# twosigma/Cook

Hardware: AMD Instinct MI355X
Metric: match-cycles/sec at 1M pending x 50k offers (higher is better)
Workload: dtype f64

## Files before the change

cook_amd/csrc/considerable_host.hpp:

```cpp
#pragma once

struct ConsWork {
  DArr<uint64_t> ukey;
  DArr<uint32_t> permA, permB, g_user, seg_start, seg_end, inexact, rate_limited, passed, qitemA, qitemB;
  DArr<uint8_t> head;
  DArr<SumU4> g_use, pre, quseA, quseB, pusage;
  DArr<int> flag1, keep_q;
  DArr<SumI> scan;
  uint32_t* result = nullptr;
  unsigned n_result = 0;
};

struct ConsBufs : ConsWork {
  bool users_staged = false;
  unsigned U = 0;
  DArr<double> qcount, qcpus, qmem, qgpus, ucount, ucpus, umem, ugpus;
  DArr<int64_t> tokens;
  bool has_tokens = false;
  int enforce = 0;
  bool has_pool_quota = false, pool_usage_given = false;
  cook_usage pool_quota{}, pool_usage{};
  bool cycle_on = false;
  DArr<uint8_t> elig_by_pending;
  bool has_elig_by_pending = false;
  DArr<double> q_cpus, q_mem, q_gpus;
  DArr<uint32_t> q_user;
  DArr<uint8_t> q_elig;
};

void cons_stage_users(cook_engine* e, ConsBufs& c, const cook_user_state* us) {
  if (!us) e->fail(COOK_E_INVALID, "cook_considerable: null user state");
  const unsigned U = us->n;
  limiter_check_user_state(e, us);
  if (U && (!us->quota_count || !us->quota_cpus || !us->quota_mem || !us->quota_gpus || !us->usage_count || !us->usage_cpus ||
            !us->usage_mem || !us->usage_gpus))
    e->fail(COOK_E_INVALID, "cook_considerable: user quota / usage arrays are required");
  c.U = U;
  h2d(e, c.qcount, us->quota_count, U);
  h2d(e, c.qcpus, us->quota_cpus, U);
  h2d(e, c.qmem, us->quota_mem, U);
  h2d(e, c.qgpus, us->quota_gpus, U);
  h2d(e, c.ucount, us->usage_count, U);
  h2d(e, c.ucpus, us->usage_cpus, U);
  h2d(e, c.umem, us->usage_mem, U);
  h2d(e, c.ugpus, us->usage_gpus, U);
  c.has_tokens = us->tokens_left != nullptr;
  if (c.has_tokens) h2d(e, c.tokens, us->tokens_left, U);
  c.enforce = us->enforce_rate_limit;
  c.has_pool_quota = us->has_pool_quota != 0;
  c.pool_quota = us->pool_quota;
  c.pool_usage_given = us->pool_usage_given != 0;
  c.pool_usage = us->pool_usage;
  sync(e);
  c.users_staged = true;
}

enum LimUse { LIM_NONE, LIM_CYCLE, LIM_READ };
void cons_run_device(cook_engine* e, const ConsBufs& s, ConsWork& c, unsigned n, const double* q_cpus, const double* q_mem,
                     const double* q_gpus, const uint32_t* q_user, const uint8_t* q_elig, unsigned K, LimUse limiters = LIM_NONE) {
  const unsigned U = s.U;
  const LimView lim = limiters != LIM_NONE ? limiter_view(e, U, limiters == LIM_CYCLE) : LimView{};
  const bool lim_commit = limiters == LIM_CYCLE && lim.tokens;
  c.rate_limited.ensure(std::max(1u, U));
  c.passed.ensure(std::max(1u, U));
  memset_async(e, c.rate_limited.ptr(), 0, (size_t)std::max(1u, U) * 4);
  memset_async(e, c.passed.ptr(), 0, (size_t)std::max(1u, U) * 4);
  c.n_result = 0;
  c.result = c.qitemA.ensure(std::max(1u, n));
  if (n == 0) return;
  const unsigned gN = div_up(n, 256);
  c.ukey.ensure(n);
  c.permA.ensure(n);
  c.permB.ensure(n);
  KM<cons_user_keys, 256>(e, "cons_user_keys", gN, q_user, n, c.ukey.ptr());
  KM<iota_u32, 256>(e, "iota", gN, c.permA.ptr(), n);
  unsigned long long umask = 0;
  for (unsigned long long x = U ? U - 1 : 0; x; x >>= 1) umask = (umask << 1) | 1ull;
  const uint32_t* permU = radix_sort_masked(e, c.ukey.ptr(), umask, c.permA.ptr(), c.permA.ptr(), c.permB.ptr(), n);
  c.g_user.ensure(n);
  c.g_use.ensure(n);
  c.head.ensure(n);
  c.seg_start.ensure(std::max(1u, U));
  c.seg_end.ensure(std::max(1u, U));
  c.inexact.ensure(std::max(1u, U));
  c.pre.ensure(n);
  memset_async(e, c.inexact.ptr(), 0, (size_t)std::max(1u, U) * 4);
  KM<cons_gather, 256>(e, "cons_gather", gN, permU, n, q_user, q_cpus, q_mem, q_gpus, c.g_user.ptr(), c.g_use.ptr(), c.head.ptr(), c.seg_start.ptr(),
      c.seg_end.ptr());
  LoadUserSeeded ld{c.g_use.ptr(), c.head.ptr(), c.g_user.ptr(), s.ucount.ptr(), s.ucpus.ptr(), s.umem.ptr(), s.ugpus.ptr()};
  seg_scan<SumU4>(e, "cons_user_usage_scan", ld, (const uint8_t*)c.head.ptr(), n, c.pre.ptr(), e->tmpU4);
  KM<rank_mark_inexact, 256>(e, "rank_mark_inexact", gN, (const SumU4*)c.pre.ptr(), (const uint32_t*)c.g_user.ptr(), n, c.inexact.ptr());
  KM<cons_fix_inexact, 256>(e, "cons_fix_inexact", div_up(std::max(1u, U), 256), (const SumU4*)c.g_use.ptr(), c.pre.ptr(),
      (const uint32_t*)c.seg_start.ptr(), (const uint32_t*)c.seg_end.ptr(), (const uint32_t*)c.inexact.ptr(), U, (const double*)s.ucount.ptr(),
      (const double*)s.ucpus.ptr(), (const double*)s.umem.ptr(), (const double*)s.ugpus.ptr());
  c.flag1.ensure(n);
  c.keep_q.ensure(n);
  c.scan.ensure(n);
  KM<cons_user_quota_flag, 256>(e, "cons_user_quota_flag", gN, (const SumU4*)c.pre.ptr(), (const uint32_t*)c.g_user.ptr(), n,
      (const double*)s.qcount.ptr(), (const double*)s.qcpus.ptr(), (const double*)s.qmem.ptr(), (const double*)s.qgpus.ptr(), c.flag1.ptr());
  seg_scan<SumI>(e, "cons_user_index_scan", LoadI{c.flag1.ptr()}, (const uint8_t*)c.head.ptr(), n, c.scan.ptr(), e->tmpI);
  unsigned* dlen = e->d_counters.ptr() + LIM_F_LEN;
  const unsigned f_words = lim_commit ? LIM_F_WORDS : 1u;
  memset_async(e, dlen, 0, f_words * 4);
  KM<cons_rate_limit, 256>(e, "cons_rate_limit", gN, (const int*)c.flag1.ptr(), (const SumI*)c.scan.ptr(), (const uint32_t*)c.g_user.ptr(), permU, n,
      s.has_tokens ? (const int64_t*)s.tokens.ptr() : (const int64_t*)nullptr, lim, s.enforce, c.keep_q.ptr(), c.rate_limited.ptr(), c.passed.ptr());
  if (lim_commit) limiter_commit_earn(e, lim, U, c.passed.ptr(), c.rate_limited.ptr(), e->d_counters.ptr());
  uint32_t* qitem = c.qitemA.ensure(n);
  uint32_t* qitem_o = c.qitemB.ensure(n);
  SumU4* quse = c.quseA.ensure(n);
  SumU4* quse_o = c.quseB.ensure(n);
  seg_scan<SumI>(e, "cons_compact_scan", LoadI{c.keep_q.ptr()}, (const uint8_t*)nullptr, n, c.scan.ptr(), e->tmpI);
  KM<cons_compact_queue, 256>(e, "cons_compact_queue", gN, (const int*)c.keep_q.ptr(), (const SumI*)c.scan.ptr(), n, q_cpus, q_mem, q_gpus, qitem, quse, dlen);
  cook_usage base = s.pool_usage;
  if (s.has_pool_quota && !s.pool_usage_given) {
    c.pusage.ensure(1);
    if (U) {
      KM<cons_pool_usage, 1024>(e, "cons_pool_usage", 1, (const double*)s.ucount.ptr(), (const double*)s.ucpus.ptr(), (const double*)s.umem.ptr(),
          (const double*)s.ugpus.ptr(), U, c.pusage.ptr());
      pinned_copy(e, e->h_scratch + 8, c.pusage.ptr(), sizeof(SumU4), hipMemcpyDeviceToHost);
    }
  }
  pinned_copy(e, e->h_scratch, dlen, f_words * 4, hipMemcpyDeviceToHost);
  sync(e);
  unsigned len = 0;
  std::memcpy(&len, e->h_scratch, 4);
  if (lim_commit) limiter_filter_finish(e, (const unsigned*)e->h_scratch);
  if (s.has_pool_quota && !s.pool_usage_given) {
    SumU4 h = SumU4::zero();
    if (U) std::memcpy(&h, e->h_scratch + 8, sizeof(SumU4));
    base = cook_usage{h.count, h.cpus, h.mem, h.gpus};
  }
  if (len && s.has_pool_quota) len = queue_filter_quota(e, 2, len, s.pool_quota, base, qitem, quse, qitem_o, quse_o);
  if (len && q_elig) {
    e->iflag.ensure(len);
    e->scanI.ensure(len);
    KM<cons_eligible_flag, 256>(e, "cons_eligible_flag", div_up(len, 256), (const uint32_t*)qitem, len, q_elig, e->iflag.ptr());
    seg_scan<SumI>(e, "queue_compact_scan", LoadI{e->iflag.ptr()}, (const uint8_t*)nullptr, len, e->scanI.ptr(), e->tmpI);
    unsigned* len_out = e->d_counters.ptr() + 9;
    KM<queue_compact, 256>(e, "queue_compact", div_up(len, 256), (const uint32_t*)qitem, (const SumU4*)quse, (const int*)e->iflag.ptr(),
        (const SumI*)e->scanI.ptr(), len, qitem_o, quse_o, len_out);
    pinned_copy(e, e->h_scratch, len_out, 4, hipMemcpyDeviceToHost);
    sync(e);
    std::memcpy(&len, e->h_scratch, 4);
    std::swap(qitem, qitem_o);
    std::swap(quse, quse_o);
  }
  c.result = qitem;
  c.n_result = std::min(len, K);
}
```

cook_amd/csrc/considerable_kernels.hpp:

```cpp
#pragma once
#include "common.hpp"
#include "scan.hpp"
#include "limiter_kernels.hpp"

COOK_KERNEL void cons_user_keys(const uint32_t* __restrict__ user, unsigned n, uint64_t* __restrict__ key) {
  const unsigned i = blockIdx.x * blockDim.x + threadIdx.x;
  if (i < n) key[i] = user[i];
}

COOK_KERNEL void cons_gather_queue(const uint32_t* __restrict__ ranked, const uint32_t* __restrict__ pend_ord,
                                                         unsigned n, const double* __restrict__ j_cpus, const double* __restrict__ j_mem,
                                                         const double* __restrict__ j_gpus, const uint32_t* __restrict__ j_user,
                                                         const uint8_t* __restrict__ elig_by_pending, double* __restrict__ q_cpus,
                                                         double* __restrict__ q_mem, double* __restrict__ q_gpus,
                                                         uint32_t* __restrict__ q_user, uint8_t* __restrict__ q_elig) {
  const unsigned q = blockIdx.x * blockDim.x + threadIdx.x;
  if (q >= n) return;
  const unsigned jj = pend_ord[ranked[q]];
  q_cpus[q] = j_cpus[jj];
  q_mem[q] = j_mem[jj];
  q_gpus[q] = j_gpus ? j_gpus[jj] : 0.0;
  q_user[q] = j_user[jj];
  q_elig[q] = elig_by_pending ? elig_by_pending[jj] : 1;
}

COOK_KERNEL void cons_gather(const uint32_t* __restrict__ permU, unsigned n, const uint32_t* __restrict__ user,
                                                   const double* __restrict__ cpus, const double* __restrict__ mem,
                                                   const double* __restrict__ gpus, uint32_t* __restrict__ g_user,
                                                   SumU4* __restrict__ g_use, uint8_t* __restrict__ head,
                                                   uint32_t* __restrict__ seg_start, uint32_t* __restrict__ seg_end) {
  const unsigned i = blockIdx.x * blockDim.x + threadIdx.x;
  if (i >= n) return;
  const unsigned t = permU[i];
  const unsigned u = user[t];
  g_user[i] = u;
  g_use[i] = SumU4{1.0, cpus[t], mem[t], gpus ? gpus[t] : 0.0, 0u};
  const bool h = (i == 0) || (user[permU[i - 1]] != u);
  head[i] = h ? 1 : 0;
  if (h) seg_start[u] = i;
  if (i == n - 1 || user[permU[i + 1]] != u) seg_end[u] = i + 1;
}

struct LoadUserSeeded {
  const SumU4* use;
  const uint8_t* head;
  const uint32_t* g_user;
  const double *uc, *ucpus, *umem, *ugpus;
  __device__ __forceinline__ SumU4 operator()(unsigned i) const {
    const SumU4 x = use[i];
    if (!head[i]) return x;
    const unsigned u = g_user[i];
    return combine(x, SumU4{uc[u], ucpus[u], umem[u], ugpus[u], 0u});
  }
};

COOK_KERNEL void cons_fix_inexact(const SumU4* __restrict__ g_use, SumU4* __restrict__ pre,
                                                        const uint32_t* __restrict__ seg_start, const uint32_t* __restrict__ seg_end,
                                                        const uint32_t* __restrict__ inexact_user, unsigned n_users,
                                                        const double* __restrict__ uc, const double* __restrict__ ucpus,
                                                        const double* __restrict__ umem, const double* __restrict__ ugpus) {
// ... 119 lines not shown
```

cook_amd/csrc/rank_host.hpp:

```cpp

template <class T, class Load>
void seg_scan(cook_engine* e, const char* tag, Load load, const uint8_t* head, unsigned n, T* out, ScanTmp<T>& tmp) {
  if (n == 0) return;
  const unsigned nb = div_up(n, SS_TILE);
  tmp.agg.ensure(nb);
  tmp.carry.ensure(nb);
  tmp.first_head.ensure(nb);
  KM<seg_scan_local<T, Load>, SS_THREADS>(e, tag, nb, load, head, n, out, tmp.agg.ptr(), tmp.first_head.ptr());
  if (nb > 1 && nb <= (unsigned)SS_THREADS) {
    KM<seg_scan_propagate_fused<T>, SS_THREADS>(e, "seg_scan_propagate", nb, out, n, (const SegAgg<T>*)tmp.agg.ptr(), (const unsigned*)tmp.first_head.ptr());
  } else if (nb > 1) {
    KM<seg_scan_blocksums<T>, SS_THREADS>(e, "seg_scan_blocksums", 1, (const SegAgg<T>*)tmp.agg.ptr(), nb, tmp.carry.ptr());
    KM<seg_scan_propagate<T>, SS_THREADS>(e, "seg_scan_propagate", nb, out, n, (const SegAgg<T>*)tmp.carry.ptr(), (const unsigned*)tmp.first_head.ptr());
  }
}

template <int IPL>
static void radix_pass_t(cook_engine* e, const uint64_t* key, const uint32_t* in, uint32_t* out, unsigned n, unsigned shift, bool fused,
                         DArr<uint32_t>& hist) {
  const unsigned nb = div_up(n, rs_tile(IPL));
  hist.ensure((size_t)256 * nb);
  KM<radix_hist<IPL>, RS_THREADS>(e, "radix_hist", nb, key, in, n, shift, nb, fused ? 1u : 0u, hist.ptr());
  if (!fused) KM<excl_scan_u32_single, SCAN1_THREADS>(e, "radix_scan", 1, hist.ptr(), 256u * nb, (uint32_t*)nullptr);
  KM<radix_scatter<IPL>, RS_THREADS>(e, "radix_scatter", nb, key, in, out, n, shift, nb, fused ? 1u : 0u, (const uint32_t*)hist.ptr());
}
void radix_pass(cook_engine* e, const uint64_t* key, const uint32_t* in, uint32_t* out, unsigned n, unsigned shift, DArr<uint32_t>& hist) {
  if (div_up(n, rs_tile(RS_IPL_SMALL)) <= RS_FUSED_BLOCKS) radix_pass_t<RS_IPL_SMALL>(e, key, in, out, n, shift, true, hist);
  else radix_pass_t<RS_IPL_LARGE>(e, key, in, out, n, shift, div_up(n, rs_tile(RS_IPL_LARGE)) <= RS_FUSED_BLOCKS_LARGE, hist);
}
uint32_t* radix_sort_masked(cook_engine* e, const uint64_t* key, unsigned long long mask, const uint32_t* cur, uint32_t* a,
                            uint32_t* b, unsigned n, DArr<uint32_t>* hist = nullptr) {
  const uint32_t* in = cur;
  uint32_t* last = const_cast<uint32_t*>(cur);
  while (mask) {
    const unsigned shift = (unsigned)__builtin_ctzll(mask);
    uint32_t* out = (in == a) ? b : a;
    radix_pass(e, key, in, out, n, shift, hist ? *hist : e->hist);
    in = out;
    last = out;
    mask = shift + 8 >= 64 ? 0ull : mask & ~((1ull << (shift + 8)) - 1ull);
  }
  return last;
}

COOK_KERNEL void iota_u32(uint32_t* p, unsigned n) {
  const unsigned i = blockIdx.x * blockDim.x + threadIdx.x;
  if (i < n) p[i] = i;
}

void rank_stage(cook_engine* e, const cook_tasks* t, const cook_users* u) {
  if (!t || !u) e->fail(COOK_E_INVALID, "cook_rank_stage: null tasks/users");
  const unsigned N = t->n, U = u->n;
  if (N && (!t->cpus || !t->mem || !t->user || !t->priority || !t->start_ms || !t->task_id || !t->job_id || !t->pending))
    e->fail(COOK_E_INVALID, "cook_rank_stage: a required task array is NULL");
  if (U == 0 && N) e->fail(COOK_E_INVALID, "cook_rank_stage: no users");
  unsigned np = 0;
  std::vector<uint32_t> pend_ord(N ? N : 1);
  for (unsigned i = 0; i < N; ++i) {
    if (t->user[i] >= U) e->fail(COOK_E_INVALID, "cook_rank_stage: user id out of range");
    pend_ord[i] = np;
    np += t->pending[i] ? 1u : 0u;
  }
  e->rank_staged = false, e->pool_usage_known = false, e->rank_done = false;
  e->hash_set = 0;
  e->N = N;
  e->U = U;
  e->n_pending = np;
  e->has_gpus = t->gpus != nullptr;
  h2d(e, e->t_cpus, t->cpus, N);
  h2d(e, e->t_mem, t->mem, N);
  if (t->gpus) h2d(e, e->t_gpus, t->gpus, N);
  h2d(e, e->t_user, t->user, N);
  h2d(e, e->t_prio, t->priority, N);
  h2d(e, e->t_start, t->start_ms, N);
  h2d(e, e->t_task, t->task_id, N);
  h2d(e, e->t_job, t->job_id, N);
  h2d(e, e->t_pending, t->pending, N);
  e->has_t_host = e->t_host_complete = t->host != nullptr;
  if (t->host) h2d(e, e->t_host, t->host, N);
  h2d(e, e->pend_ord, pend_ord.data(), N);
  h2d(e, e->u_divc, u->div_cpus, U);
  h2d(e, e->u_divm, u->div_mem, U);
  h2d(e, e->u_divg, u->div_gpus, U);
  h2d(e, e->u_qcount, u->quota_count, U);
  h2d(e, e->u_qcpus, u->quota_cpus, U);
  h2d(e, e->u_qmem, u->quota_mem, U);
  h2d(e, e->u_qgpus, u->quota_gpus, U);
  sync(e);
  e->rank_staged = true;
  e->pool_usage_known = false;
  e->rank_done = false;
}

void rank_pool_usage(cook_engine* e, cook_usage* out) {
  if (!e->rank_staged) e->fail(COOK_E_STATE, "cook_rank_pool_usage before cook_rank_stage");
  static const bool memo = [] { const char* v = std::getenv("COOK_POOL_USAGE_MEMO"); return !(v && v[0] == '0'); }();
  if (e->pool_usage_known && memo) {
    *out = e->pool_usage_val;
    return;
  }
  e->pool_usage.ensure(1);
  if (e->N == 0) {
    *out = cook_usage{0, 0, 0, 0};
    return;
  }
  e->pool_usage.ensure(1 + POOL_USAGE_BLOCKS);
  e->pool_usage_bound.ensure(POOL_USAGE_BLOCKS);
  KM<pool_usage_partial, 256>(e, "pool_usage_partial", POOL_USAGE_BLOCKS, (const double*)e->t_cpus.ptr(), (const double*)e->t_mem.ptr(),
      e->has_gpus ? (const double*)e->t_gpus.ptr() : (const double*)nullptr, (const uint8_t*)e->t_pending.ptr(), e->N, e->pool_usage.ptr() + 1,
      e->pool_usage_bound.ptr(), (unsigned)POOL_USAGE_BLOCKS);
  KM<pool_usage_reduce, COOK_WAVE>(e, "pool_usage_reduce", 1, (const double*)e->t_cpus.ptr(), (const double*)e->t_mem.ptr(),
      e->has_gpus ? (const double*)e->t_gpus.ptr() : (const double*)nullptr, (const uint8_t*)e->t_pending.ptr(), e->N,
      (const SumU4*)(e->pool_usage.ptr() + 1), (const SumBound4*)e->pool_usage_bound.ptr(), (unsigned)POOL_USAGE_BLOCKS, e->pool_usage.ptr());
  SumU4 h;
  pinned_copy(e, e->h_scratch, e->pool_usage.ptr(), sizeof(SumU4), hipMemcpyDeviceToHost);
  sync(e);
  std::memcpy(&h, e->h_scratch, sizeof(SumU4));
  *out = cook_usage{h.count, h.cpus, h.mem, h.gpus};
  e->pool_usage_val = *out;
  e->pool_usage_known = true;
}

void rank_user_usage(cook_engine* e, double* out, bool out_is_device) {
  if (!e->rank_done) e->fail(COOK_E_STATE, "cook_rank_user_usage before cook_rank_run");
  if (!out) e->fail(COOK_E_INVALID, "cook_rank_user_usage: null output");
  const unsigned N = e->N, U = e->U;
  if (U == 0) return;
  double* dst = out_is_device ? out : e->uu_out.ensure((size_t)U * 3);
  if (N) {
    SumU4* rp = e->uu_pre.ensure(N);
    uint32_t* bad = e->uu_bad.ensure(U);
    memset_async(e, bad, 0, (size_t)U * 4);
    seg_scan<SumU4>(e, "user_running_scan", LoadRunningU4{e->s_use.ptr(), e->s_pending.ptr()}, (const uint8_t*)e->head.ptr(), N, rp,
                    e->tmpU4);
    KM<rank_mark_inexact, 256>(e, "user_usage_mark", div_up(N, 256), (const SumU4*)rp, (const uint32_t*)e->s_user.ptr(), N, bad);
    KM<user_usage_extract, 256>(e, "user_usage_extract", div_up(U, 256), (const SumU4*)rp, (const SumU4*)e->s_use.ptr(),
        (const uint8_t*)e->s_pending.ptr(), (const uint32_t*)e->seg_start.ptr(), (const uint32_t*)e->seg_end.ptr(), (const uint32_t*)bad, U, dst);
  } else {
    memset_async(e, dst, 0, (size_t)U * 24);
  }
  if (!out_is_device) copy_async(e, out, dst, (size_t)U * 24, hipMemcpyDeviceToHost);
  sync(e);
}

unsigned queue_filter_quota(cook_engine* e, unsigned stage, unsigned len, const cook_usage& quota, const cook_usage& base, uint32_t*& qitem,
                            SumU4*& quse, uint32_t*& qitem_other, SumU4*& quse_other) {
  if (len == 0) return 0;
  e->qpre.ensure(len);
  e->iflag.ensure(len);
  e->scanI.ensure(len);
  LoadQueueUse ld{quse, SumU4{base.count, base.cpus, base.mem, base.gpus, 0u}};
  seg_scan<SumU4>(e, "queue_usage_scan", ld, (const uint8_t*)nullptr, len, e->qpre.ptr(), e->tmpU4);
  unsigned* any_bad = e->d_counters.ptr() + 32 + 2 * stage;
  if (stage >= 2) memset_async(e, any_bad, 0, 8);
  Usage4 q{quota.count, quota.cpus, quota.mem, quota.gpus};
  KM<queue_quota_flag, 256>(e, "queue_quota_flag", div_up(len, 256), (const SumU4*)e->qpre.ptr(), len, q, e->iflag.ptr(), any_bad);
  KM<queue_quota_fix, 64>(e, "queue_quota_fix", 1, (const SumU4*)quse, len, SumU4{base.count, base.cpus, base.mem, base.gpus, 0u}, q,
      (const unsigned*)any_bad, e->iflag.ptr());
  seg_scan<SumI>(e, "queue_compact_scan", LoadI{e->iflag.ptr()}, (const uint8_t*)nullptr, len, e->scanI.ptr(), e->tmpI);
  unsigned* len_out = any_bad + 1;
  KM<queue_compact, 256>(e, "queue_compact", div_up(len, 256), (const uint32_t*)qitem, (const SumU4*)quse, (const int*)e->iflag.ptr(),
      (const SumI*)e->scanI.ptr(), len, qitem_other, quse_other, len_out);
  unsigned h[2];
  pinned_copy(e, e->h_scratch, len_out, 4, hipMemcpyDeviceToHost);
  sync(e);
  std::memcpy(h, e->h_scratch, 4);
  std::swap(qitem, qitem_other);
  std::swap(quse, quse_other);
  return h[0];
}

void rank_run(cook_engine* e) {
  if (!e->rank_staged) e->fail(COOK_E_STATE, "cook_rank_run before cook_rank_stage");
  const auto t_call = std::chrono::steady_clock::now();
  if (g_sync_trace) tl_sync_ms = 0.0, tl_syncs = 0;
  const unsigned N = e->N, U = e->U;
  e->n_ranked = 0;
  e->rank_done = false;
  e->cycle_cons_ran = false;
  e->q_valid = false;
  e->q_stepped = false;
  e->ranked.ensure(std::max(1u, e->n_pending));
  if (N == 0) {
    e->rank_done = true;
    return;
  }
  const unsigned gN = div_up(N, 256);
  e->d_scratch64.ensure(64);
  e->d_counters.ensure(64);
  const bool radix_only = std::getenv("COOK_RANK_RADIX") != nullptr;
  unsigned long long* mins = e->d_scratch64.ptr();
  unsigned long long* same = e->d_scratch64.ptr() + 4;
  e->seg_start.ensure(U);
  e->seg_end.ensure(U);
  e->inexact_user.ensure(U);
  TieCtl* tie_ctl0 = e->tie_ctl.ensure(1);
  bool tie_ctl_clean = true;
  KM<rank_init, 256>(e, "rank_init", std::max(1u, std::min(div_up(U, 256), 64u)), e->d_scratch64.ptr(), e->d_counters.ptr(), 40u,
      e->inexact_user.ptr(), e->seg_end.ptr(), U, reinterpret_cast<unsigned*>(tie_ctl0), (unsigned)(sizeof(TieCtl) / 4), std::max(1u,
      std::min(div_up(U, 256), 64u)));
  e->w0.ensure(N);
  e->w1.ensure(N);
  e->w2.ensure(N);
  KM<rank_key_mins, 256>(e, "rank_key_mins", std::min(gN, 64u), (const int64_t*)e->t_start.ptr(), (const int64_t*)e->t_task.ptr(),
      (const int64_t*)e->t_job.ptr(), (const uint8_t*)e->t_pending.ptr(), N, mins, std::min(gN, 64u));
  KM<rank_build_keys, 256>(e, "rank_build_keys", gN, (const uint32_t*)e->t_user.ptr(), (const int32_t*)e->t_prio.ptr(),
      (const int64_t*)e->t_start.ptr(), (const int64_t*)e->t_task.ptr(), (const int64_t*)e->t_job.ptr(), (const uint8_t*)e->t_pending.ptr(), N,
// ... 235 lines not shown
```

cook_amd/csrc/rank_kernels.hpp:

```cpp
#pragma once
#include "common.hpp"
#include "scan.hpp"

COOK_KERNEL void rank_init(unsigned long long* __restrict__ scratch64, unsigned* __restrict__ counters, unsigned n_counters,
                                                 uint32_t* __restrict__ inexact_user, uint32_t* __restrict__ seg_end, unsigned n_users,
                                                 unsigned* __restrict__ tie_ctl, unsigned tie_ctl_words, unsigned nblk ) {
  const unsigned i = blockIdx.x * blockDim.x + threadIdx.x;
  if (i < 7) scratch64[i] = ~0ull;
  if (i < n_counters) counters[i] = 0u;
  if (i < tie_ctl_words) tie_ctl[i] = 0u;
  for (unsigned u = i; u < n_users; u += nblk * blockDim.x) {
    inexact_user[u] = 0u;
    seg_end[u] = 0u;
  }
}

COOK_KERNEL void rank_key_mins(const int64_t* __restrict__ start_ms, const int64_t* __restrict__ task_id,
                                                     const int64_t* __restrict__ job_id, const uint8_t* __restrict__ pending,
                                                     unsigned n, unsigned long long* __restrict__ mins , unsigned nblk) {
  unsigned long long m0 = ~0ull, m1 = ~0ull, m2 = ~0ull;
  for (unsigned i = blockIdx.x * blockDim.x + threadIdx.x; i < n; i += nblk * blockDim.x) {
    if (pending[i]) {
      const unsigned long long k = i64_key(job_id[i]);
      m1 = k < m1 ? k : m1;
// ... 356 lines not shown
    cp = x.cpus + cp;
    m = x.mem + m;
    g = x.gpus + g;
    flag[q] = below_quota4(quota.count, quota.cpus, quota.mem, quota.gpus, Usage4{c, cp, m, g}) ? 1 : 0;
  }
}

COOK_KERNEL void queue_offensive_flag(const SumU4* __restrict__ quse, unsigned len, double max_mem, double max_cpus,
                                                            int* __restrict__ flag) {
  const unsigned q = blockIdx.x * blockDim.x + threadIdx.x;
  if (q >= len) return;
  const SumU4 x = quse[q];
  flag[q] = (x.mem > max_mem || x.cpus > max_cpus) ? 0 : 1;
}

COOK_KERNEL void queue_compact(const uint32_t* __restrict__ qitem_in, const SumU4* __restrict__ quse_in,
                                                     const int* __restrict__ flag, const SumI* __restrict__ incl, unsigned len,
                                                     uint32_t* __restrict__ qitem_out, SumU4* __restrict__ quse_out,
                                                     unsigned* __restrict__ len_out) {
  const unsigned q = blockIdx.x * blockDim.x + threadIdx.x;
  if (q >= len) return;
  if (flag[q]) {
    const unsigned o = (unsigned)incl[q].v - 1;
    qitem_out[o] = qitem_in[q];
    quse_out[o] = quse_in[q];
  }
  if (q == len - 1) *len_out = (unsigned)incl[q].v;
}

COOK_KERNEL void queue_emit(const uint32_t* __restrict__ qitem, unsigned len, const uint32_t* __restrict__ permB,
                                                  uint32_t* __restrict__ ranked) {
  const unsigned q = blockIdx.x * blockDim.x + threadIdx.x;
  if (q < len) ranked[q] = permB[qitem[q]];
}
COOK_KERNEL void dru_to_task_space(const double* __restrict__ dru, const uint8_t* __restrict__ keep,
                                                         const uint32_t* __restrict__ permB, unsigned n, double* __restrict__ out) {
  const unsigned i = blockIdx.x * blockDim.x + threadIdx.x;
  if (i < n) out[permB[i]] = keep[i] ? dru[i] : __longlong_as_double(0x7FF8000000000000ll);
}

struct LoadRunningU4 {
  const SumU4* use;
  const uint8_t* pending;
  __device__ __forceinline__ SumU4 operator()(unsigned i) const {
    if (pending[i]) return SumU4::zero();
    SumU4 x = use[i];
    if (__double_as_longlong(x.cpus) == LLONG_MIN || __double_as_longlong(x.mem) == LLONG_MIN || __double_as_longlong(x.gpus) == LLONG_MIN)
      x.bad = 1u;
    return x;
  }
};
COOK_KERNEL void user_usage_extract(const SumU4* __restrict__ run_pre, const SumU4* __restrict__ s_use,
                                                          const uint8_t* __restrict__ s_pending, const uint32_t* __restrict__ seg_start,
                                                          const uint32_t* __restrict__ seg_end, const uint32_t* __restrict__ inexact_user,
                                                          unsigned n_users, double* __restrict__ out ) {
  const unsigned u = blockIdx.x * blockDim.x + threadIdx.x;
  if (u >= n_users) return;
  double c = 0.0, m = 0.0, g = 0.0;
  if (seg_end[u] != 0u) {
    const unsigned a = seg_start[u], b = seg_end[u];
    const SumU4 t = run_pre[b - 1];
    if (!inexact_user[u]) {
      c = t.cpus, m = t.mem, g = t.gpus;
    } else {
      bool first = true;
      for (unsigned i = a; i < b; ++i) {
        if (s_pending[i]) continue;
        const SumU4 x = s_use[i];
        if (first) {
          c = x.cpus, m = x.mem, g = x.gpus;
          first = false;
        } else {
          c += x.cpus, m += x.mem, g += x.gpus;
        }
      }
    }
  }
  out[(size_t)u * 3 + 0] = c;
  out[(size_t)u * 3 + 1] = m;
  out[(size_t)u * 3 + 2] = g;
}
constexpr int POOL_USAGE_BLOCKS = 64;
COOK_KERNEL void pool_usage_partial(const double* __restrict__ cpus, const double* __restrict__ mem,
                                                          const double* __restrict__ gpus, const uint8_t* __restrict__ pending,
                                                          unsigned n, SumU4* __restrict__ part, SumBound4* __restrict__ part_bound, unsigned nblk) {
  __shared__ SumU4 ws[256 / COOK_WAVE];
  __shared__ SumBound4 wb[256 / COOK_WAVE];
  SumU4 acc = SumU4::zero();
  SumBound4 bd = SumBound4::zero();
  for (unsigned i = blockIdx.x * blockDim.x + threadIdx.x; i < n; i += nblk * blockDim.x)
    if (!pending[i]) {
      const double x[4] = {1.0, cpus[i], mem[i], gpus ? gpus[i] : 0.0};
      acc = combine(acc, SumU4{x[0], x[1], x[2], x[3], 0u});
      bound_add(bd, x);
    }
  for (int d = 32; d >= 1; d >>= 1) {
    SumU4 o;
    o.count = __shfl_xor(acc.count, d, COOK_WAVE);
    o.cpus = __shfl_xor(acc.cpus, d, COOK_WAVE);
    o.mem = __shfl_xor(acc.mem, d, COOK_WAVE);
    o.gpus = __shfl_xor(acc.gpus, d, COOK_WAVE);
    o.bad = __shfl_xor(acc.bad, d, COOK_WAVE);
    acc = combine(acc, o);
    bound_merge(bd, bound_shfl_xor(bd, d));
  }
  if (lane_id() == 0) ws[wave_id()] = acc, wb[wave_id()] = bd;
  __syncthreads();
  if (threadIdx.x == 0) {
    SumU4 t = ws[0];
    SumBound4 tb = wb[0];
    for (unsigned k = 1; k < blockDim.x / COOK_WAVE; ++k) t = combine(t, ws[k]), bound_merge(tb, wb[k]);
    part[blockIdx.x] = t;
    part_bound[blockIdx.x] = tb;
  }
}
// ... 26 lines not shown
```

cook_amd/csrc/sort.hpp:

```cpp
#pragma once
#include "common.hpp"

constexpr int RS_THREADS = 256;
constexpr int RS_WAVES = RS_THREADS / COOK_WAVE;
constexpr int RS_IPL_LARGE = 16;
constexpr int RS_IPL_SMALL = 8;
constexpr unsigned RS_FUSED_BLOCKS = COOK_SHAPE(128, 2);
constexpr unsigned RS_FUSED_BLOCKS_LARGE = COOK_SHAPE(512, 3);
constexpr unsigned rs_tile(int ipl) { return (unsigned)(RS_WAVES * COOK_WAVE * ipl); }

static __device__ __forceinline__ unsigned rs_digit(const uint64_t* __restrict__ key, const uint32_t* __restrict__ perm_in,
                                                    unsigned i, unsigned shift) {
  const unsigned src = perm_in ? perm_in[i] : i;
  return (unsigned)(key[src] >> shift) & 0xFFu;
}

template <int IPL>
COOK_KERNEL void radix_hist(const uint64_t* __restrict__ key, const uint32_t* __restrict__ perm_in,
                                                         unsigned n, unsigned shift, unsigned nblocks, unsigned fused,
                                                         uint32_t* __restrict__ hist) {
  __shared__ unsigned h[256];
  h[threadIdx.x] = 0;
  __syncthreads();
  const unsigned base = blockIdx.x * rs_tile(IPL);
  unsigned d[rs_tile(IPL) / RS_THREADS];
#pragma unroll
  for (unsigned k = 0; k < rs_tile(IPL) / RS_THREADS; ++k) {
    const unsigned i = base + k * RS_THREADS + threadIdx.x;
    d[k] = i < n ? rs_digit(key, perm_in, i, shift) : 0xFFFFFFFFu;
  }
#pragma unroll
  for (unsigned k = 0; k < rs_tile(IPL) / RS_THREADS; ++k)
    if (d[k] != 0xFFFFFFFFu) atomicAdd(&h[d[k]], 1u);
  __syncthreads();
  hist[fused ? blockIdx.x * 256u + threadIdx.x : threadIdx.x * nblocks + blockIdx.x] = h[threadIdx.x];
}

constexpr int SCAN1_THREADS = 1024;
constexpr int SCAN1_IPT = 8;
constexpr int SCAN1_NS = 8;
static_assert(SCAN1_IPT == 8, "a thread moves its entries as two 16-byte vectors");
COOK_KERNEL void excl_scan_u32_single(uint32_t* __restrict__ data, unsigned len,
                                                                      uint32_t* __restrict__ total_out) {
  __shared__ unsigned wsum[2][SCAN1_THREADS / COOK_WAVE];
  unsigned carry = 0;
  const unsigned lane = lane_id(), w = wave_id();
  constexpr unsigned STEP = SCAN1_THREADS * SCAN1_IPT;
  for (unsigned super = 0; super < len; super += STEP * SCAN1_NS) {
    unsigned v[SCAN1_NS][SCAN1_IPT];
#pragma unroll
    for (int s = 0; s < SCAN1_NS; ++s) {
      const unsigned i0 = super + (unsigned)s * STEP + threadIdx.x * SCAN1_IPT;
      if (i0 + SCAN1_IPT <= len) {
        const uint4 a = *reinterpret_cast<const uint4*>(data + i0), b = *reinterpret_cast<const uint4*>(data + i0 + 4);
        v[s][0] = a.x, v[s][1] = a.y, v[s][2] = a.z, v[s][3] = a.w;
        v[s][4] = b.x, v[s][5] = b.y, v[s][6] = b.z, v[s][7] = b.w;
      } else {
#pragma unroll
        for (int q = 0; q < SCAN1_IPT; ++q) v[s][q] = i0 + q < len ? data[i0 + q] : 0u;
      }
    }
#pragma unroll
    for (int s = 0; s < SCAN1_NS; ++s) {
      if (super + (unsigned)s * STEP >= len) break;
      const unsigned i0 = super + (unsigned)s * STEP + threadIdx.x * SCAN1_IPT;
      unsigned tot = 0;
#pragma unroll
      for (int q = 0; q < SCAN1_IPT; ++q) tot += v[s][q];
      unsigned inc = tot;
      for (unsigned d = 1; d < COOK_WAVE; d <<= 1) {
        const unsigned t = __shfl_up(inc, d, COOK_WAVE);
        if (lane >= d) inc += t;
      }
      if (lane == COOK_WAVE - 1) wsum[s & 1][w] = inc;
      __syncthreads();
      unsigned wbase = 0, all = 0;
      for (unsigned k = 0; k < SCAN1_THREADS / COOK_WAVE; ++k) {
        const unsigned x = wsum[s & 1][k];
        wbase += k < w ? x : 0u;
        all += x;
      }
      unsigned run = carry + wbase + inc - tot;
      unsigned o[SCAN1_IPT];
#pragma unroll
      for (int q = 0; q < SCAN1_IPT; ++q) {
        o[q] = run;
        run += v[s][q];
      }
      if (i0 + SCAN1_IPT <= len) {
        *reinterpret_cast<uint4*>(data + i0) = uint4{o[0], o[1], o[2], o[3]};
        *reinterpret_cast<uint4*>(data + i0 + 4) = uint4{o[4], o[5], o[6], o[7]};
      } else {
#pragma unroll
        for (int q = 0; q < SCAN1_IPT; ++q)
          if (i0 + q < len) data[i0 + q] = o[q];
      }
      carry += all;
    }
  }
  if (total_out && threadIdx.x == 0) *total_out = carry;
}

template <int IPL>
COOK_KERNEL void radix_scatter(const uint64_t* __restrict__ key, const uint32_t* __restrict__ perm_in,
                                                            uint32_t* __restrict__ perm_out, unsigned n, unsigned shift,
                                                            unsigned nblocks, unsigned fused, const uint32_t* __restrict__ hist) {
  __shared__ unsigned whist[RS_WAVES][256];
  __shared__ unsigned wtot[RS_WAVES];
  __shared__ uint4 s_tot[RS_WAVES][COOK_WAVE], s_bel[RS_WAVES][COOK_WAVE];
  const unsigned lane = lane_id(), w = wave_id();
  for (int k = 0; k < RS_WAVES; ++k) whist[k][threadIdx.x] = 0;
  unsigned below = 0, total = 0;
  if (fused) {
    uint4 tot{0u, 0u, 0u, 0u}, bel{0u, 0u, 0u, 0u};
#pragma unroll 8
    for (unsigned t = w; t < nblocks; t += RS_WAVES) {
      const uint4 v = *reinterpret_cast<const uint4*>(hist + (size_t)t * 256u + 4u * lane);
      tot.x += v.x, tot.y += v.y, tot.z += v.z, tot.w += v.w;
      if (t < blockIdx.x) bel.x += v.x, bel.y += v.y, bel.z += v.z, bel.w += v.w;
    }
    s_tot[w][lane] = tot;
    s_bel[w][lane] = bel;
  }
  __syncthreads();
  if (fused) {
    const unsigned* pt = reinterpret_cast<const unsigned*>(&s_tot[0][0]);
    const unsigned* pb = reinterpret_cast<const unsigned*>(&s_bel[0][0]);
    for (int k = 0; k < RS_WAVES; ++k) {
      total += pt[k * 256 + threadIdx.x];
      below += pb[k * 256 + threadIdx.x];
    }
  }
  const unsigned wbase = blockIdx.x * rs_tile(IPL) + w * (COOK_WAVE * IPL);
  unsigned src[IPL], dg[IPL];
#pragma unroll
  for (int k = 0; k < IPL; ++k) {
    const unsigned i = wbase + k * COOK_WAVE + lane;
    src[k] = i < n ? (perm_in ? perm_in[i] : i) : 0xFFFFFFFFu;
  }
#pragma unroll
  for (int k = 0; k < IPL; ++k) dg[k] = src[k] != 0xFFFFFFFFu ? (unsigned)(key[src[k]] >> shift) & 0xFFu : 0u;
#pragma unroll
  for (int k = 0; k < IPL; ++k)
    if (src[k] != 0xFFFFFFFFu) atomicAdd(&whist[w][dg[k]], 1u);
  if (fused) {
    unsigned inc = total;
    for (unsigned d = 1; d < COOK_WAVE; d <<= 1) {
      const unsigned t = __shfl_up(inc, d, COOK_WAVE);
      if (lane >= d) inc += t;
    }
    if (lane == COOK_WAVE - 1) wtot[w] = inc;
    __syncthreads();
    unsigned before = 0;
    for (unsigned k = 0; k < (unsigned)RS_WAVES; ++k) before += k < w ? wtot[k] : 0u;
    below += before + inc - total;
  } else {
    __syncthreads();
    below = hist[threadIdx.x * nblocks + blockIdx.x];
  }
  {
    unsigned base = below;
    for (int k = 0; k < RS_WAVES; ++k) {
      const unsigned t = whist[k][threadIdx.x];
      whist[k][threadIdx.x] = base;
      base += t;
    }
  }
  __syncthreads();
  const unsigned long long lt = lanemask_lt();
#pragma unroll
  for (int k = 0; k < IPL; ++k) {
    const bool valid = src[k] != 0xFFFFFFFFu;
    const unsigned d = dg[k];
    unsigned long long peers = __ballot(valid);
    for (int b = 0; b < 8; ++b) {
      const unsigned long long m = __ballot(valid && ((d >> b) & 1u));
      peers &= ((d >> b) & 1u) ? m : ~m;
    }
    unsigned slot = 0;
    if (valid) slot = whist[w][d];
    wave_sync();
    if (valid) {
      const unsigned rank = (unsigned)__popcll(peers & lt);
      if (rank == 0) whist[w][d] = slot + (unsigned)__popcll(peers);
      perm_out[slot + rank] = src[k];
    }
    wave_sync();
  }
}

COOK_KERNEL void radix_varying_bits(const uint64_t* __restrict__ key, unsigned n,
                                                          unsigned long long* __restrict__ out_mask, unsigned nblk) {
  const uint64_t k0 = key[0];
  unsigned long long m = 0;
  for (unsigned i = blockIdx.x * blockDim.x + threadIdx.x; i < n; i += nblk * blockDim.x) m |= key[i] ^ k0;
  for (int d = 32; d >= 1; d >>= 1) m |= __shfl_xor(m, d, COOK_WAVE);
  __shared__ unsigned long long s_m[256 / COOK_WAVE];
  if (lane_id() == 0) s_m[wave_id()] = m;
  __syncthreads();
  if (threadIdx.x == 0) {
    unsigned long long b = 0ull;
    for (unsigned w = 0; w < blockDim.x / COOK_WAVE; ++w) b |= s_m[w];
    if (b) atomicOr(out_mask, b);
  }
}
```

Measured before the change: 23.07.

## Fold memsets into key kernel, widen radix digits to 9 bits, lazy-clear flags

```diff
diff --git a/cook_amd/csrc/considerable_host.hpp b/cook_amd/csrc/considerable_host.hpp
--- a/cook_amd/csrc/considerable_host.hpp
+++ b/cook_amd/csrc/considerable_host.hpp
@@ -56,6 +56,7 @@
 }
 
 enum LimUse { LIM_NONE, LIM_CYCLE, LIM_READ };
+constexpr unsigned CONS_CLEAR_FROM = 36, CONS_CLEAR_WORDS = 11;
 void cons_run_device(cook_engine* e, const ConsBufs& s, ConsWork& c, unsigned n, const double* q_cpus, const double* q_mem,
                      const double* q_gpus, const uint32_t* q_user, const uint8_t* q_elig, unsigned K, LimUse limiters = LIM_NONE) {
   const unsigned U = s.U;
@@ -63,16 +64,21 @@
   const bool lim_commit = limiters == LIM_CYCLE && lim.tokens;
   c.rate_limited.ensure(std::max(1u, U));
   c.passed.ensure(std::max(1u, U));
-  memset_async(e, c.rate_limited.ptr(), 0, (size_t)std::max(1u, U) * 4);
-  memset_async(e, c.passed.ptr(), 0, (size_t)std::max(1u, U) * 4);
   c.n_result = 0;
   c.result = c.qitemA.ensure(std::max(1u, n));
-  if (n == 0) return;
+  if (n == 0) {
+    memset_async(e, c.rate_limited.ptr(), 0, (size_t)std::max(1u, U) * 4);
+    memset_async(e, c.passed.ptr(), 0, (size_t)std::max(1u, U) * 4);
+    return;
+  }
   const unsigned gN = div_up(n, 256);
   c.ukey.ensure(n);
   c.permA.ensure(n);
   c.permB.ensure(n);
-  KM<cons_user_keys, 256>(e, "cons_user_keys", gN, q_user, n, c.ukey.ptr());
+  c.inexact.ensure(std::max(1u, U));
+  static_assert(CONS_CLEAR_FROM + CONS_CLEAR_WORDS == LIM_F_LEN + LIM_F_WORDS && CONS_CLEAR_WORDS <= 256, "one thread per cleared counter");
+  KM<cons_user_keys, 256>(e, "cons_user_keys", gN, q_user, n, c.ukey.ptr(), c.rate_limited.ptr(), c.passed.ptr(), c.inexact.ptr(), std::max(1u, U),
+      e->d_counters.ptr() + CONS_CLEAR_FROM, CONS_CLEAR_WORDS, gN);
   KM<iota_u32, 256>(e, "iota", gN, c.permA.ptr(), n);
   unsigned long long umask = 0;
   for (unsigned long long x = U ? U - 1 : 0; x; x >>= 1) umask = (umask << 1) | 1ull;
@@ -82,9 +88,7 @@
   c.head.ensure(n);
   c.seg_start.ensure(std::max(1u, U));
   c.seg_end.ensure(std::max(1u, U));
-  c.inexact.ensure(std::max(1u, U));
   c.pre.ensure(n);
-  memset_async(e, c.inexact.ptr(), 0, (size_t)std::max(1u, U) * 4);
   KM<cons_gather, 256>(e, "cons_gather", gN, permU, n, q_user, q_cpus, q_mem, q_gpus, c.g_user.ptr(), c.g_use.ptr(), c.head.ptr(), c.seg_start.ptr(),
       c.seg_end.ptr());
   LoadUserSeeded ld{c.g_use.ptr(), c.head.ptr(), c.g_user.ptr(), s.ucount.ptr(), s.ucpus.ptr(), s.umem.ptr(), s.ugpus.ptr()};
@@ -101,7 +105,6 @@
   seg_scan<SumI>(e, "cons_user_index_scan", LoadI{c.flag1.ptr()}, (const uint8_t*)c.head.ptr(), n, c.scan.ptr(), e->tmpI);
   unsigned* dlen = e->d_counters.ptr() + LIM_F_LEN;
   const unsigned f_words = lim_commit ? LIM_F_WORDS : 1u;
-  memset_async(e, dlen, 0, f_words * 4);
   KM<cons_rate_limit, 256>(e, "cons_rate_limit", gN, (const int*)c.flag1.ptr(), (const SumI*)c.scan.ptr(), (const uint32_t*)c.g_user.ptr(), permU, n,
       s.has_tokens ? (const int64_t*)s.tokens.ptr() : (const int64_t*)nullptr, lim, s.enforce, c.keep_q.ptr(), c.rate_limited.ptr(), c.passed.ptr());
   if (lim_commit) limiter_commit_earn(e, lim, U, c.passed.ptr(), c.rate_limited.ptr(), e->d_counters.ptr());
diff --git a/cook_amd/csrc/considerable_kernels.hpp b/cook_amd/csrc/considerable_kernels.hpp
--- a/cook_amd/csrc/considerable_kernels.hpp
+++ b/cook_amd/csrc/considerable_kernels.hpp
@@ -3,9 +3,18 @@
 #include "scan.hpp"
 #include "limiter_kernels.hpp"
 
-COOK_KERNEL void cons_user_keys(const uint32_t* __restrict__ user, unsigned n, uint64_t* __restrict__ key) {
+COOK_KERNEL void cons_user_keys(const uint32_t* __restrict__ user, unsigned n, uint64_t* __restrict__ key,
+                                                      uint32_t* __restrict__ rate_limited, uint32_t* __restrict__ passed,
+                                                      uint32_t* __restrict__ inexact, unsigned n_users, unsigned* __restrict__ counters,
+                                                      unsigned n_counters, unsigned nblk ) {
   const unsigned i = blockIdx.x * blockDim.x + threadIdx.x;
   if (i < n) key[i] = user[i];
+  if (i < n_counters) counters[i] = 0u;
+  for (unsigned u = i; u < n_users; u += nblk * blockDim.x) {
+    rate_limited[u] = 0u;
+    passed[u] = 0u;
+    inexact[u] = 0u;
+  }
 }
 
 COOK_KERNEL void cons_gather_queue(const uint32_t* __restrict__ ranked, const uint32_t* __restrict__ pend_ord,
diff --git a/cook_amd/csrc/rank_host.hpp b/cook_amd/csrc/rank_host.hpp
--- a/cook_amd/csrc/rank_host.hpp
+++ b/cook_amd/csrc/rank_host.hpp
@@ -15,30 +15,46 @@
   }
 }
 
-template <int IPL>
+template <int IPL, int BITS>
 static void radix_pass_t(cook_engine* e, const uint64_t* key, const uint32_t* in, uint32_t* out, unsigned n, unsigned shift, bool fused,
                          DArr<uint32_t>& hist) {
   const unsigned nb = div_up(n, rs_tile(IPL));
-  hist.ensure((size_t)256 * nb);
-  KM<radix_hist<IPL>, RS_THREADS>(e, "radix_hist", nb, key, in, n, shift, nb, fused ? 1u : 0u, hist.ptr());
-  if (!fused) KM<excl_scan_u32_single, SCAN1_THREADS>(e, "radix_scan", 1, hist.ptr(), 256u * nb, (uint32_t*)nullptr);
-  KM<radix_scatter<IPL>, RS_THREADS>(e, "radix_scatter", nb, key, in, out, n, shift, nb, fused ? 1u : 0u, (const uint32_t*)hist.ptr());
-}
-void radix_pass(cook_engine* e, const uint64_t* key, const uint32_t* in, uint32_t* out, unsigned n, unsigned shift, DArr<uint32_t>& hist) {
-  if (div_up(n, rs_tile(RS_IPL_SMALL)) <= RS_FUSED_BLOCKS) radix_pass_t<RS_IPL_SMALL>(e, key, in, out, n, shift, true, hist);
-  else radix_pass_t<RS_IPL_LARGE>(e, key, in, out, n, shift, div_up(n, rs_tile(RS_IPL_LARGE)) <= RS_FUSED_BLOCKS_LARGE, hist);
+  hist.ensure(((size_t)1 << BITS) * nb);
+  KM<radix_hist<IPL, BITS>, RS_THREADS>(e, "radix_hist", nb, key, in, n, shift, nb, fused ? 1u : 0u, hist.ptr());
+  if (!fused) KM<excl_scan_u32_single, SCAN1_THREADS>(e, "radix_scan", 1, hist.ptr(), (1u << BITS) * nb, (uint32_t*)nullptr);
+  KM<radix_scatter<IPL, BITS>, RS_THREADS>(e, "radix_scatter", nb, key, in, out, n, shift, nb, fused ? 1u : 0u, (const uint32_t*)hist.ptr());
+}
+template <int BITS>
+static void radix_pass_b(cook_engine* e, const uint64_t* key, const uint32_t* in, uint32_t* out, unsigned n, unsigned shift, DArr<uint32_t>& hist) {
+  if (div_up(n, rs_tile(RS_IPL_SMALL)) <= RS_FUSED_BLOCKS) radix_pass_t<RS_IPL_SMALL, BITS>(e, key, in, out, n, shift, true, hist);
+  else radix_pass_t<RS_IPL_LARGE, BITS>(e, key, in, out, n, shift, div_up(n, rs_tile(RS_IPL_LARGE)) <= RS_FUSED_BLOCKS_LARGE, hist);
+}
+void radix_pass(cook_engine* e, const uint64_t* key, const uint32_t* in, uint32_t* out, unsigned n, unsigned shift, unsigned bits,
+                DArr<uint32_t>& hist) {
+  static_assert(RS_BITS_MIN == 8 && RS_BITS_MAX == 9, "one instantiation per digit width");
+  if (bits <= 8) radix_pass_b<8>(e, key, in, out, n, shift, hist);
+  else radix_pass_b<9>(e, key, in, out, n, shift, hist);
+}
+constexpr size_t RS_HIST_ENTRIES_MAX = (size_t)COOK_SHAPE(512, 16) << RS_BITS_MIN;
+static unsigned radix_digit_bits(unsigned n) {
+  const unsigned small = div_up(n, rs_tile(RS_IPL_SMALL));
+  const unsigned nb = small <= RS_FUSED_BLOCKS ? small : div_up(n, rs_tile(RS_IPL_LARGE));
+  unsigned bits = RS_BITS_MAX;
+  while (bits > (unsigned)RS_BITS_MIN && ((size_t)nb << bits) > RS_HIST_ENTRIES_MAX) --bits;
+  return bits;
 }
 uint32_t* radix_sort_masked(cook_engine* e, const uint64_t* key, unsigned long long mask, const uint32_t* cur, uint32_t* a,
                             uint32_t* b, unsigned n, DArr<uint32_t>* hist = nullptr) {
   const uint32_t* in = cur;
   uint32_t* last = const_cast<uint32_t*>(cur);
+  const unsigned bits = radix_digit_bits(n);
   while (mask) {
     const unsigned shift = (unsigned)__builtin_ctzll(mask);
     uint32_t* out = (in == a) ? b : a;
-    radix_pass(e, key, in, out, n, shift, hist ? *hist : e->hist);
+    radix_pass(e, key, in, out, n, shift, bits, hist ? *hist : e->hist);
     in = out;
     last = out;
-    mask = shift + 8 >= 64 ? 0ull : mask & ~((1ull << (shift + 8)) - 1ull);
+    mask = shift + bits >= 64 ? 0ull : mask & ~((1ull << (shift + bits)) - 1ull);
   }
   return last;
 }
@@ -129,13 +145,14 @@
   double* dst = out_is_device ? out : e->uu_out.ensure((size_t)U * 3);
   if (N) {
     SumU4* rp = e->uu_pre.ensure(N);
+    const bool fresh = e->uu_bad.b.cap < (size_t)U * 4;
     uint32_t* bad = e->uu_bad.ensure(U);
-    memset_async(e, bad, 0, (size_t)U * 4);
+    if (fresh) memset_async(e, bad, 0, e->uu_bad.b.cap);
     seg_scan<SumU4>(e, "user_running_scan", LoadRunningU4{e->s_use.ptr(), e->s_pending.ptr()}, (const uint8_t*)e->head.ptr(), N, rp,
                     e->tmpU4);
     KM<rank_mark_inexact, 256>(e, "user_usage_mark", div_up(N, 256), (const SumU4*)rp, (const uint32_t*)e->s_user.ptr(), N, bad);
     KM<user_usage_extract, 256>(e, "user_usage_extract", div_up(U, 256), (const SumU4*)rp, (const SumU4*)e->s_use.ptr(),
-        (const uint8_t*)e->s_pending.ptr(), (const uint32_t*)e->seg_start.ptr(), (const uint32_t*)e->seg_end.ptr(), (const uint32_t*)bad, U, dst);
+        (const uint8_t*)e->s_pending.ptr(), (const uint32_t*)e->seg_start.ptr(), (const uint32_t*)e->seg_end.ptr(), bad, U, dst);
   } else {
     memset_async(e, dst, 0, (size_t)U * 24);
   }
@@ -152,7 +169,6 @@
   LoadQueueUse ld{quse, SumU4{base.count, base.cpus, base.mem, base.gpus, 0u}};
   seg_scan<SumU4>(e, "queue_usage_scan", ld, (const uint8_t*)nullptr, len, e->qpre.ptr(), e->tmpU4);
   unsigned* any_bad = e->d_counters.ptr() + 32 + 2 * stage;
-  if (stage >= 2) memset_async(e, any_bad, 0, 8);
   Usage4 q{quota.count, quota.cpus, quota.mem, quota.gpus};
   KM<queue_quota_flag, 256>(e, "queue_quota_flag", div_up(len, 256), (const SumU4*)e->qpre.ptr(), len, q, e->iflag.ptr(), any_bad);
   KM<queue_quota_fix, 64>(e, "queue_quota_fix", 1, (const SumU4*)quse, len, SumU4{base.count, base.cpus, base.mem, base.gpus, 0u}, q,
diff --git a/cook_amd/csrc/rank_kernels.hpp b/cook_amd/csrc/rank_kernels.hpp
--- a/cook_amd/csrc/rank_kernels.hpp
+++ b/cook_amd/csrc/rank_kernels.hpp
@@ -432,15 +432,17 @@
 };
 COOK_KERNEL void user_usage_extract(const SumU4* __restrict__ run_pre, const SumU4* __restrict__ s_use,
                                                           const uint8_t* __restrict__ s_pending, const uint32_t* __restrict__ seg_start,
-                                                          const uint32_t* __restrict__ seg_end, const uint32_t* __restrict__ inexact_user,
+                                                          const uint32_t* __restrict__ seg_end, uint32_t* __restrict__ inexact_user,
                                                           unsigned n_users, double* __restrict__ out ) {
   const unsigned u = blockIdx.x * blockDim.x + threadIdx.x;
   if (u >= n_users) return;
+  const uint32_t inexact = inexact_user[u];
+  if (inexact) inexact_user[u] = 0u;
   double c = 0.0, m = 0.0, g = 0.0;
   if (seg_end[u] != 0u) {
     const unsigned a = seg_start[u], b = seg_end[u];
     const SumU4 t = run_pre[b - 1];
-    if (!inexact_user[u]) {
+    if (!inexact) {
       c = t.cpus, m = t.mem, g = t.gpus;
     } else {
       bool first = true;
diff --git a/cook_amd/csrc/sort.hpp b/cook_amd/csrc/sort.hpp
--- a/cook_amd/csrc/sort.hpp
+++ b/cook_amd/csrc/sort.hpp
@@ -9,31 +9,39 @@
 constexpr unsigned RS_FUSED_BLOCKS_LARGE = COOK_SHAPE(512, 3);
 constexpr unsigned rs_tile(int ipl) { return (unsigned)(RS_WAVES * COOK_WAVE * ipl); }
 
+constexpr int RS_BITS_MIN = 8, RS_BITS_MAX = 9;
+
 static __device__ __forceinline__ unsigned rs_digit(const uint64_t* __restrict__ key, const uint32_t* __restrict__ perm_in,
-                                                    unsigned i, unsigned shift) {
+                                                    unsigned i, unsigned shift, unsigned dmask) {
   const unsigned src = perm_in ? perm_in[i] : i;
-  return (unsigned)(key[src] >> shift) & 0xFFu;
-}
-
-template <int IPL>
+  return (unsigned)(key[src] >> shift) & dmask;
+}
+
+template <int IPL, int BITS>
 COOK_KERNEL void radix_hist(const uint64_t* __restrict__ key, const uint32_t* __restrict__ perm_in,
                                                          unsigned n, unsigned shift, unsigned nblocks, unsigned fused,
                                                          uint32_t* __restrict__ hist) {
-  __shared__ unsigned h[256];
-  h[threadIdx.x] = 0;
+  constexpr unsigned D = 1u << BITS;
+  __shared__ unsigned h[D];
+#pragma unroll
+  for (unsigned q = 0; q < D / RS_THREADS; ++q) h[q * RS_THREADS + threadIdx.x] = 0;
   __syncthreads();
   const unsigned base = blockIdx.x * rs_tile(IPL);
   unsigned d[rs_tile(IPL) / RS_THREADS];
 #pragma unroll
   for (unsigned k = 0; k < rs_tile(IPL) / RS_THREADS; ++k) {
     const unsigned i = base + k * RS_THREADS + threadIdx.x;
-    d[k] = i < n ? rs_digit(key, perm_in, i, shift) : 0xFFFFFFFFu;
+    d[k] = i < n ? rs_digit(key, perm_in, i, shift, D - 1u) : 0xFFFFFFFFu;
   }
 #pragma unroll
   for (unsigned k = 0; k < rs_tile(IPL) / RS_THREADS; ++k)
     if (d[k] != 0xFFFFFFFFu) atomicAdd(&h[d[k]], 1u);
   __syncthreads();
-  hist[fused ? blockIdx.x * 256u + threadIdx.x : threadIdx.x * nblocks + blockIdx.x] = h[threadIdx.x];
+#pragma unroll
+  for (unsigned q = 0; q < D / RS_THREADS; ++q) {
+    const unsigned dg = q * RS_THREADS + threadIdx.x;
+    hist[fused ? blockIdx.x * D + dg : dg * nblocks + blockIdx.x] = h[dg];
+  }
 }
 
 constexpr int SCAN1_THREADS = 1024;
@@ -101,35 +109,51 @@
   if (total_out && threadIdx.x == 0) *total_out = carry;
 }
 
-template <int IPL>
+template <int IPL, int BITS>
 COOK_KERNEL void radix_scatter(const uint64_t* __restrict__ key, const uint32_t* __restrict__ perm_in,
                                                             uint32_t* __restrict__ perm_out, unsigned n, unsigned shift,
                                                             unsigned nblocks, unsigned fused, const uint32_t* __restrict__ hist) {
-  __shared__ unsigned whist[RS_WAVES][256];
+  constexpr unsigned D = 1u << BITS, J = D / RS_THREADS;
+  constexpr unsigned CH = D / (4u * COOK_WAVE);
+  constexpr unsigned NPART = CH >= RS_WAVES ? 1u : RS_WAVES / CH;
+  constexpr unsigned CPW = CH >= RS_WAVES ? CH / RS_WAVES : 1u;
+  static_assert(BITS >= RS_BITS_MIN && BITS <= RS_BITS_MAX && (CH * NPART == RS_WAVES || CPW * RS_WAVES == CH), "digit widths of the kernels");
+  __shared__ unsigned whist[RS_WAVES][D];
   __shared__ unsigned wtot[RS_WAVES];
-  __shared__ uint4 s_tot[RS_WAVES][COOK_WAVE], s_bel[RS_WAVES][COOK_WAVE];
+  __shared__ uint4 s_tot[NPART][D / 4u], s_bel[NPART][D / 4u];
   const unsigned lane = lane_id(), w = wave_id();
-  for (int k = 0; k < RS_WAVES; ++k) whist[k][threadIdx.x] = 0;
-  unsigned below = 0, total = 0;
+#pragma unroll
+  for (unsigned q = 0; q < J; ++q)
+    for (int k = 0; k < RS_WAVES; ++k) whist[k][q * RS_THREADS + threadIdx.x] = 0;
+  unsigned below[J], total[J];
+#pragma unroll
+  for (unsigned q = 0; q < J; ++q) below[q] = 0, total[q] = 0;
   if (fused) {
-    uint4 tot{0u, 0u, 0u, 0u}, bel{0u, 0u, 0u, 0u};
+    const unsigned part = NPART > 1u ? w / CH : 0u;
+#pragma unroll
+    for (unsigned c = 0; c < CPW; ++c) {
+      const unsigned chunk = NPART > 1u ? w % CH : w + c * RS_WAVES;
+      uint4 tot{0u, 0u, 0u, 0u}, bel{0u, 0u, 0u, 0u};
 #pragma unroll 8
-    for (unsigned t = w; t < nblocks; t += RS_WAVES) {
-      const uint4 v = *reinterpret_cast<const uint4*>(hist + (size_t)t * 256u + 4u * lane);
-      tot.x += v.x, tot.y += v.y, tot.z += v.z, tot.w += v.w;
-      if (t < blockIdx.x) bel.x += v.x, bel.y += v.y, bel.z += v.z, bel.w += v.w;
-    }
-    s_tot[w][lane] = tot;
-    s_bel[w][lane] = bel;
+      for (unsigned t = part; t < nblocks; t += NPART) {
+        const uint4 v = *reinterpret_cast<const uint4*>(hist + (size_t)t * D + 4u * (chunk * COOK_WAVE + lane));
+        tot.x += v.x, tot.y += v.y, tot.z += v.z, tot.w += v.w;
+        if (t < blockIdx.x) bel.x += v.x, bel.y += v.y, bel.z += v.z, bel.w += v.w;
+      }
+      s_tot[part][chunk * COOK_WAVE + lane] = tot;
+      s_bel[part][chunk * COOK_WAVE + lane] = bel;
+    }
   }
   __syncthreads();
   if (fused) {
     const unsigned* pt = reinterpret_cast<const unsigned*>(&s_tot[0][0]);
     const unsigned* pb = reinterpret_cast<const unsigned*>(&s_bel[0][0]);
-    for (int k = 0; k < RS_WAVES; ++k) {
-      total += pt[k * 256 + threadIdx.x];
-      below += pb[k * 256 + threadIdx.x];
-    }
+    for (unsigned k = 0; k < NPART; ++k)
+#pragma unroll
+      for (unsigned q = 0; q < J; ++q) {
+        total[q] += pt[k * D + J * threadIdx.x + q];
+        below[q] += pb[k * D + J * threadIdx.x + q];
+      }
   }
   const unsigned wbase = blockIdx.x * rs_tile(IPL) + w * (COOK_WAVE * IPL);
   unsigned src[IPL], dg[IPL];
@@ -139,12 +163,15 @@
     src[k] = i < n ? (perm_in ? perm_in[i] : i) : 0xFFFFFFFFu;
   }
 #pragma unroll
-  for (int k = 0; k < IPL; ++k) dg[k] = src[k] != 0xFFFFFFFFu ? (unsigned)(key[src[k]] >> shift) & 0xFFu : 0u;
+  for (int k = 0; k < IPL; ++k) dg[k] = src[k] != 0xFFFFFFFFu ? (unsigned)(key[src[k]] >> shift) & (D - 1u) : 0u;
 #pragma unroll
   for (int k = 0; k < IPL; ++k)
     if (src[k] != 0xFFFFFFFFu) atomicAdd(&whist[w][dg[k]], 1u);
   if (fused) {
-    unsigned inc = total;
+    unsigned tsum = 0;
+#pragma unroll
+    for (unsigned q = 0; q < J; ++q) tsum += total[q];
+    unsigned inc = tsum;
     for (unsigned d = 1; d < COOK_WAVE; d <<= 1) {
       const unsigned t = __shfl_up(inc, d, COOK_WAVE);
       if (lane >= d) inc += t;
@@ -153,16 +180,23 @@
     __syncthreads();
     unsigned before = 0;
     for (unsigned k = 0; k < (unsigned)RS_WAVES; ++k) before += k < w ? wtot[k] : 0u;
-    below += before + inc - total;
+    unsigned run = before + inc - tsum;
+#pragma unroll
+    for (unsigned q = 0; q < J; ++q) {
+      below[q] += run;
+      run += total[q];
+    }
   } else {
     __syncthreads();
-    below = hist[threadIdx.x * nblocks + blockIdx.x];
-  }
-  {
-    unsigned base = below;
+#pragma unroll
+    for (unsigned q = 0; q < J; ++q) below[q] = hist[(J * threadIdx.x + q) * nblocks + blockIdx.x];
+  }
+#pragma unroll
+  for (unsigned q = 0; q < J; ++q) {
+    unsigned base = below[q];
     for (int k = 0; k < RS_WAVES; ++k) {
-      const unsigned t = whist[k][threadIdx.x];
-      whist[k][threadIdx.x] = base;
+      const unsigned t = whist[k][J * threadIdx.x + q];
+      whist[k][J * threadIdx.x + q] = base;
       base += t;
     }
   }
@@ -173,7 +207,8 @@
     const bool valid = src[k] != 0xFFFFFFFFu;
     const unsigned d = dg[k];
     unsigned long long peers = __ballot(valid);
-    for (int b = 0; b < 8; ++b) {
+#pragma unroll
+    for (int b = 0; b < BITS; ++b) {
       const unsigned long long m = __ballot(valid && ((d >> b) & 1u));
       peers &= ((d >> b) & 1u) ? m : ~m;
     }
```

After: 23.17 (median of 2 runs). No clear change (+0.4%).
